# zhen6618/EPRecon

Hardware: AMD Instinct MI355X
Metric: fragments_per_sec (higher is better)
Workload: dtype f32

## Files before the change

### eprecon_amd/_lib.py

```python
import ctypes
import os

import torch

_HERE = os.path.dirname(os.path.abspath(__file__))
LIB_PATH = os.environ.get("EPRECON_LIB_PATH") or os.path.join(_HERE, "libeprecon_hip.so")

_c = ctypes
_vp, _i, _i64, _f, _sz = _c.c_void_p, _c.c_int, _c.c_int64, _c.c_float, _c.c_size_t

SIGNATURES = {
    "eprecon_abi_version": (_i, []),
    "eprecon_build_arch": (_c.c_char_p, []),
    "eprecon_back_project_workspace_bytes": (_sz, [_i64, _i, _i, _i, _i, _i, _i]),
    "eprecon_back_project_async": (_i, [_vp, _i64, _vp, _i, _f, _vp, _i, _vp, _i, _i, _i, _i, _i, _i,
                                        _vp, _vp, _vp, _vp, _vp, _vp, _vp, _vp, _sz, _vp]),
    "eprecon_back_project": (_i, [_vp, _i64, _vp, _i, _f, _vp, _i, _vp, _i, _i, _i, _i, _i, _i, _i,
                                  _vp, _vp, _vp, _vp, _vp, _vp, _vp, _vp, _vp, _sz, _vp]),
    "eprecon_profile_gather_kernel": (_c.c_char_p, []),
    "eprecon_hash_capacity": (_c.c_uint32, [_i64]),
    "eprecon_hash_table_bytes": (_sz, [_c.c_uint32]),
    "eprecon_hash_build_async": (_i, [_vp, _i64, _i, _vp, _c.c_uint32, _vp]),
    "eprecon_hash_build_dn_async": (_i, [_vp, _i64, _vp, _i, _vp, _c.c_uint32, _vp]),
    "eprecon_hash_query_async": (_i, [_vp, _c.c_uint32, _vp, _i64, _i, _vp, _vp]),
# ... 13 lines not shown
    "eprecon_transpose_map_async": (_i, [_vp, _i64, _vp, _i, _vp, _vp]),
    "eprecon_sparse_conv_async": (_i, [_vp, _i64, _i, _vp, _i, _i64, _vp, _i, _i, _vp, _vp, _i, _i, _i, _vp]),
    "eprecon_conv_bn_partial_bytes": (_sz, [_i64, _i]),
    "eprecon_sparse_conv_fused_async": (_i, [_vp, _i64, _i, _vp, _i, _i64, _vp, _i, _i, _vp, _vp, _i, _vp, _i, _i, _i,
                                             _vp, _vp]),
    "eprecon_conv_desc_async": (_i, [_vp, _vp]),
    "eprecon_exclusive_scan_async": (_i, [_vp, _i64, _vp, _vp, _vp, _vp]),
    "eprecon_conv_desc_partial_rows": (_i64, [_vp]),
    "eprecon_bn_acc_words": (_sz, [_i]),
    "eprecon_conv_desc_takes_bn_acc": (_i, [_vp]),
    "eprecon_batchnorm_acc_affine_async": (_i, [_vp, _i, _i, _i, _f, _vp, _vp, _vp]),
    "eprecon_affine_rows_acc_async": (_i, [_vp, _i64, _i, _i, _vp, _i, _i, _f, _i, _vp, _i, _vp]),
    "eprecon_affine_rows_res_async": (_i, [_vp, _i64, _i, _i, _vp, _vp, _vp, _i, _i, _vp, _i, _vp]),
    "eprecon_batchnorm_finalize_affine_async": (_i, [_vp, _i64, _i, _vp, _vp, _f, _vp, _vp, _vp]),
    "eprecon_affine_rows_async": (_i, [_vp, _i64, _i, _i, _vp, _vp, _i, _vp, _i, _vp]),
    "eprecon_pixel_map_async": (_i, [_i, _i, _i, _i, _vp, _vp]),
    "eprecon_batchnorm_apply_workspace_bytes": (_sz, [_i]),
    "eprecon_batchnorm_apply_partials_async": (_i, [_vp, _i64, _i, _i, _vp, _i64, _vp, _vp, _f, _vp, _i, _i, _vp, _i,
                                                    _vp, _vp, _vp, _sz, _vp]),
    "eprecon_batchnorm_apply_partials_res_async": (_i, [_vp, _i64, _i, _i, _vp, _i64, _vp, _vp, _f, _vp, _i, _vp, _vp, _i, _vp,
                                                        _i, _vp, _sz, _vp]),
    "eprecon_batchnorm_workspace_bytes": (_sz, [_i64, _i]),
    "eprecon_batchnorm_train_async": (_i, [_vp, _i64, _i, _i, _vp, _vp, _f, _vp, _i, _i, _vp, _i, _vp, _vp,
                                           _vp, _sz, _vp]),
    "eprecon_rowwise_layernorm_async": (_i, [_vp, _i64, _i, _i, _vp, _i, _vp, _vp, _f, _i, _i, _vp, _i, _vp]),
    "eprecon_init_select_workspace_bytes": (_sz, [_i, _i]),
    "eprecon_init_select_async": (_i, [_vp, _vp, _i64, _f, _i, _i, _i, _vp, _vp, _vp, _sz, _vp]),
    "eprecon_upsample_async": (_i, [_vp, _i, _vp, _i64, _i, _i, _vp, _vp, _vp]),
    "eprecon_aligned_coords_async": (_i, [_vp, _i64, _vp, _i, _f, _vp, _vp, _vp]),
    "eprecon_point_quantize_async": (_i, [_vp, _i64, _f, _vp, _vp, _vp]),
# ... 155 lines not shown
                ("residual", ctypes.c_void_p), ("ld_res", ctypes.c_int),
                ("out", ctypes.c_void_p), ("ld_out", ctypes.c_int),
                ("relu", ctypes.c_int), ("accumulate", ctypes.c_int),
                ("in_scale", ctypes.c_void_p), ("in_shift", ctypes.c_void_p), ("in_relu", ctypes.c_int),
                ("res_scale", ctypes.c_void_p), ("res_shift", ctypes.c_void_p), ("res_relu", ctypes.c_int),
                ("bn_partial", ctypes.c_void_p),
                ("ln", ctypes.c_int), ("ln_gamma", ctypes.c_void_p), ("ln_beta", ctypes.c_void_p),
                ("ln_eps", ctypes.c_float), ("ln_post_relu", ctypes.c_int),
                ("img_h", ctypes.c_int), ("img_w", ctypes.c_int), ("img_maps", ctypes.c_int),
                ("vox_rank", ctypes.c_void_p), ("grid_x", ctypes.c_int), ("grid_y", ctypes.c_int), ("grid_z", ctypes.c_int),
                ("packed_weight", ctypes.c_void_p), ("packed_weight16", ctypes.c_void_p),
                ("workspace", ctypes.c_void_p), ("workspace_bytes", ctypes.c_size_t),
                ("bn_acc", ctypes.c_void_p), ("bn_acc_ld", ctypes.c_int), ("bn_acc_c0", ctypes.c_int),
                ("bn_gamma", ctypes.c_void_p), ("bn_beta", ctypes.c_void_p),
                ("in_acc", ctypes.c_void_p), ("in_acc_ld", ctypes.c_int), ("in_acc_c0", ctypes.c_int),
                ("in_eps", ctypes.c_float), ("in_affine_scratch", ctypes.c_void_p)]


class GruStageDesc(ctypes.Structure):
    _fields_ = [("map", ctypes.c_void_p), ("target_map", ctypes.c_void_p),
                ("cur_coords", ctypes.c_void_p), ("cur_feat", ctypes.c_void_p), ("n_cur", ctypes.c_int64), ("ld_cur", ctypes.c_int),
                ("dim", ctypes.c_int), ("interval", ctypes.c_int), ("activity_mode", ctypes.c_int),
                ("rel", ctypes.c_int32 * 3),
                ("tsdf_gt", ctypes.c_void_p), ("occ_gt", ctypes.c_void_p),
                ("origin", ctypes.c_void_p), ("w2ac", ctypes.c_void_p),
                ("voxel_size", ctypes.c_float), ("resolution", ctypes.c_float),
                ("ch_voxel", ctypes.c_int), ("batch_index", ctypes.c_int),
                ("capacity", ctypes.c_int64),
                ("updated", ctypes.c_void_p), ("out_coords", ctypes.c_void_p), ("r_coords", ctypes.c_void_p),
                ("hx_voxel", ctypes.c_void_p), ("hx_image", ctypes.c_void_p), ("tsdf_target", ctypes.c_void_p),
                ("scaled1", ctypes.c_void_p), ("vox1", ctypes.c_void_p), ("inverse1", ctypes.c_void_p), ("uniq1", ctypes.c_void_p),
# ... 187 lines not shown
```

### eprecon_amd/csrc/conv_common.hpp

```cpp
#pragma once
#include "common.hpp"

namespace epconv {

struct ConvParams {
    const float *x;
    const int32_t *nbr;
    const float *w;
    const float *bias;
    float *out;
    int n_out, K, Cin, Cout, ld_x, ld_out;
    int64_t x_bytes;
    int relu;
    int accumulate;
    const float *res;
    int ld_res;
    float *bn_partial;
    const float *in_scale, *in_shift;
    int in_relu;
    const float *res_scale, *res_shift;
    int res_relu;
    int ln;
    const float *ln_gamma, *ln_beta;
    float ln_eps;
// ... 2 lines not shown
    int flex_partial;
    const int32_t *vox_rank;
    int gx, gy, gz;
    const float *wq;
    const float *wq16;
    int debug;
    int splitk_pipe;
    void *ws;
    size_t ws_bytes;
    long long *bn_acc;
    int bn_acc_ld, bn_acc_c0;
    const float *bn_gamma, *bn_beta;
    const long long *in_acc;
    int in_acc_ld, in_acc_c0;
    float in_eps;
};

constexpr int kBnCopies = 8, kBnWords = 7;
#ifndef EP_BN_ABL
#define EP_BN_ABL 0
#endif

__device__ __forceinline__ void bn_limbs(double x, long long &l0, long long &l1, long long &l2)
{
    const double v = x * 1099511627776.0;
    const double hi = floor(v * (1.0 / 1099511627776.0));
    l0 = (long long)(v - hi * 1099511627776.0);
    const long long h = (long long)hi;
    l1 = h & ((1ll << 40) - 1);
    l2 = h >> 40;
// ... 90 lines not shown
```

### eprecon_amd/csrc/grid_ops.hip

```cpp
#include "common.hpp"

namespace {
using namespace ep;

constexpr int kSelThreads = 1024;

__global__ __launch_bounds__(256) void init_mark_kernel(const float *logit, const int4 *coords, int n, float thr,
                                                        int batch, int D, int cell, unsigned char *marks)
{
    const int i = blockIdx.x * 256 + threadIdx.x;
    if (i >= n) return;
    const int4 c = coords[i];
    if (c.x < 0 || c.x >= batch) return;
    const float sig = 1.0f / (1.0f + expf(-logit[i]));
    if (sig > thr) {
        const int x = c.y / cell, y = c.z / cell, z = c.w / cell;
        if (x >= 0 && x < D && y >= 0 && y < D && z >= 0 && z < D) marks[(size_t)c.x * D * D * D + (x * D + y) * D + z] = 1;
    }
}

__device__ __forceinline__ uint32_t box_columns(const uint32_t *vol, int D, int x, int y, bool erode, uint32_t zmask)
{
    uint32_t r = erode ? zmask : 0u;
    for (int dx = -1; dx <= 1; ++dx)
// ... 128 lines not shown
        hipLaunchKernelGGL(upsample_coords_kernel, dim3((unsigned)ceil_div(n * 8, 256)), dim3(256), 0, st,
                           reinterpret_cast<const int4 *>(coords), (int)n, interval,
                           reinterpret_cast<int4 *>(up_coords));
        EP_LAUNCH_CHECK();
    }
    if (channels > 0) {
        if (!feat || !up_feat || ld_feat < channels) return EPRECON_ERR_ARG;
        const size_t total = (size_t)n * 8 * channels;
        hipLaunchKernelGGL(upsample_feat_kernel, dim3((unsigned)ceil_div((int64_t)total, 256)), dim3(256), 0,
                           st, feat, (int)n, channels, ld_feat, up_feat);
        EP_LAUNCH_CHECK();
    }
    return EPRECON_OK;
}

}

namespace {
__global__ __launch_bounds__(256) void upsample2x_nhwc_kernel(const float4 *in, float4 *out, int n, int h, int w,
                                                              int c4)
{
    const size_t e = (size_t)blockIdx.x * 256 + threadIdx.x;
    const size_t total = (size_t)n * 4 * h * w * c4;
    if (e >= total) return;
    const int c = (int)(e % c4);
    size_t r = e / c4;
    const int ox = (int)(r % (2 * w));
    r /= 2 * w;
    const int oy = (int)(r % (2 * h));
    const int img = (int)(r / (2 * h));
// ... 163 lines not shown
```

### eprecon_amd/csrc/sparse_conv.hip

```cpp
#include <stdio.h>
#include <stdlib.h>
#include <string.h>

#include "common.hpp"
#include "conv_common.hpp"

namespace {
using namespace ep;
using namespace epconv;

typedef float f32x16 __attribute__((ext_vector_type(16)));


template <int TN>
__device__ __forceinline__ void stage_weights(float *dst, const float *w, int row0, int row_end, int stride,
                                              int ncols, int rows, int tid)
{
    const int total = rows * TN;
    if (stride == TN && ncols >= TN && (reinterpret_cast<uintptr_t>(w) & 15) == 0) {
        const float4 *src = reinterpret_cast<const float4 *>(w + (size_t)row0 * stride);
        float4 *d4 = reinterpret_cast<float4 *>(dst);
        const int valid4 = max(0, min(rows, row_end - row0)) * (TN / 4);
#pragma unroll 4
        for (int e = tid; e < total / 4; e += 256) d4[e] = e < valid4 ? src[min(e, max(valid4 - 1, 0))] : make_float4(0.f, 0.f, 0.f, 0.f);
// ... 1967 lines not shown
        EP_LAUNCH_CHECK();
    }
    return rc;
}

int conv_dispatch_inner(ConvParams &p, int64_t n_in, hipStream_t st)
{
    {
        const int kind = conv3d_kind(p);
        if (kind != kD3None) {
            g_last_conv_kernel = kind == kD3Narrow ? "conv3d_tile_narrow_kernel" : "conv3d_tile16_kernel";
            return kind == kD3Tile16 ? launch_conv3d_16(p, st) : launch_conv3d_single_column(p, st);
        }
        if (!p.nbr && p.K != 1) return EPRECON_ERR_ARG;
    }
    const bool direct2d = p.K == 9 && direct16_ok(p);
    if (!direct2d) {
        int nt, nch;
        int64_t blocks;
        if (conv2d_tile_ok(p, &nt, &nch, &blocks)) {
            g_last_conv_kernel = "conv2d_tile_kernel";
            switch (nch) {
                case 1: return launch_conv2d_tile<1>(p, st);
                case 2: return launch_conv2d_tile<2>(p, st);
                case 3: return launch_conv2d_tile<3>(p, st);
                case 4: return launch_conv2d_tile<4>(p, st);
                default: return launch_conv2d_tile<5>(p, st);
            }
        }
    }
// ... 137 lines not shown
extern "C" size_t eprecon_conv_bn_partial_bytes(int64_t n_out, int cout)
{
    return (size_t)ep::ceil_div(n_out > 0 ? n_out : 1, (int64_t)128) * 3 * (size_t)(cout > 0 ? cout : 1) * sizeof(float);
}

static int conv_check_and_run(ConvParams &p, int64_t n_in, int64_t n_out, void *stream)
{
    if (!p.x || !p.w || !p.out || n_in < 0 || n_out < 0 || p.K <= 0 || p.K > 64 || p.Cin <= 0 || p.Cout <= 0 ||
        p.ld_x < p.Cin || p.ld_out < p.Cout || (p.res && p.ld_res < p.Cout))
        return EPRECON_ERR_ARG;
    if (!p.nbr && !p.vox_rank && p.K != 1) return EPRECON_ERR_ARG;
    if (!p.nbr && n_in != n_out) return EPRECON_ERR_ARG;
    if ((p.in_scale == nullptr) != (p.in_shift == nullptr) || (p.res_scale == nullptr) != (p.res_shift == nullptr))
        return EPRECON_ERR_ARG;
    if (p.Cout > 4096 || n_out > 0x7fffffff) return EPRECON_ERR_UNSUPPORTED;
    if (n_out == 0) return EPRECON_OK;
    p.n_out = (int)n_out;
    p.x_bytes = n_in > 0 ? ((n_in - 1) * (int64_t)p.ld_x + ((p.Cin + 3) & ~3)) * 4 : 0;
    return conv_dispatch(p, n_in, (hipStream_t)stream);
}

static void params_from_desc(ConvParams &p, const eprecon_conv_desc *d)
{
    p.x = d->x; p.nbr = d->nbr; p.w = d->weight; p.bias = d->bias; p.out = d->out;
    p.K = d->kvol; p.Cin = d->cin; p.Cout = d->cout; p.ld_x = d->ld_x; p.ld_out = d->ld_out;
    p.relu = d->relu; p.accumulate = d->accumulate;
    p.res = d->residual; p.ld_res = d->ld_res; p.bn_partial = d->bn_partial;
    p.in_scale = d->in_scale; p.in_shift = d->in_shift; p.in_relu = d->in_relu;
    p.res_scale = d->res_scale; p.res_shift = d->res_shift; p.res_relu = d->res_relu;
    p.ln = d->ln; p.ln_gamma = d->ln_gamma; p.ln_beta = d->ln_beta; p.ln_eps = d->ln_eps;
    p.ln_post_relu = d->ln_post_relu;
    p.img_h = d->img_h; p.img_w = d->img_w; p.img_maps = d->img_maps;
    p.vox_rank = d->vox_rank; p.gx = d->grid_x; p.gy = d->grid_y; p.gz = d->grid_z; p.wq = d->packed_weight;
    p.wq16 = d->packed_weight16;
    p.ws = d->workspace; p.ws_bytes = d->workspace_bytes;
    p.flex_partial = 1;
    p.bn_acc = d->bn_acc; p.bn_acc_ld = d->bn_acc_ld; p.bn_acc_c0 = d->bn_acc_c0; p.bn_gamma = d->bn_gamma; p.bn_beta = d->bn_beta;
    p.in_acc = d->in_acc; p.in_acc_ld = d->in_acc_ld; p.in_acc_c0 = d->in_acc_c0; p.in_eps = d->in_eps;
}

extern "C" int eprecon_batchnorm_acc_affine_async(const long long *acc, int acc_ld, int acc_c0, int channels, float eps,
                                                  float *scale_out, float *shift_out, void *stream);

static bool bn_acc_family(const ConvParams &p) { return conv3d_kind(p) == 0; }

extern "C" size_t eprecon_bn_acc_words(int ld)
{
    return ld > 0 ? (size_t)epconv::kBnCopies * ld * epconv::kBnWords + (size_t)(2 * ld + 1) / 2 : 0;
}

extern "C" int eprecon_conv_desc_takes_bn_acc(const eprecon_conv_desc *d)
{
    if (!d || d->n_out <= 0) return 0;
// ... 81 lines not shown
```

### eprecon_amd/csrc/sparse_conv_direct_impl.hpp

```cpp
#pragma once
#include <stdlib.h>

#include <atomic>
#include <type_traits>

#include "common.hpp"
#include "conv_common.hpp"

namespace epconv {
namespace {
using namespace ep;

constexpr int kRT = 2;

#ifndef EP_DIRECT_ABL
#define EP_DIRECT_ABL 0
#endif

__device__ __forceinline__ float relu_nc(float x)
{
    float r;
    asm("v_max_f32 %0, 0, %1" : "=v"(r) : "v"(x));
    return r;
}
// ... 66 lines not shown
            if (colok[t] && orow[r] >= 0) {
                val = acc[r >> 2][t][r & 3] + b;
                if (p.relu) val = fmaxf(val, 0.0f);
                if (p.res) {
                    float rv = p.res[(size_t)orow[r] * p.ld_res + col];
                    if (p.res_scale) {
                        rv = fmaf(rv, rs, rb);
                        if (p.res_relu) rv = fmaxf(rv, 0.0f);
                    }
                    val += rv;
                }
            }
            v[t][r] = val;
        }
    }
    if (p.ln) {
        const float inv_c = 1.0f / (float)p.Cout;
#pragma unroll
        for (int r = 0; r < NR; ++r) {
            float sum = 0.0f;
#pragma unroll
            for (int t = 0; t < CT; ++t) sum += v[t][r];
#pragma unroll
            for (int m = 8; m > 0; m >>= 1) sum += __shfl_xor(sum, m);
            const float mean = sum * inv_c;
            float sq = 0.0f;
#pragma unroll
            for (int t = 0; t < CT; ++t) {
                const float d = colok[t] ? v[t][r] - mean : 0.0f;
                v[t][r] = d;
                sq = fmaf(d, d, sq);
// ... 840 lines not shown
        if (n <= 0) n = 256;
    }
    return n;
}

static bool persist_enabled()
{
    const char *e = getenv("EPRECON_CONV_PERSIST");
    return e && e[0] == '1';
}

constexpr int kPersistMinRows = 8192;

static bool persist_ok(const ConvParams &p)
{
    if (!persist_enabled() || (p.Cin + 15) / 16 > 6) return false;
    if (p.Cout - 16 * ((p.Cout + 15) / 16 - 1) <= 8 && !tail8_enabled()) return false;
    if (p.bn_partial && !p.flex_partial) return false;
    if (persist_lds_bytes(p) > kLdsBytes) return false;
    {
        const int kch = (p.Cin + 15) / 16, ct = (p.Cout + 15) / 16;
        const bool tail = p.Cout - 16 * (ct - 1) <= 8;
        if (kch * ((tail ? ct - 1 : ct) * 1024 + (tail ? 512 : 0)) > 4864) return false;
    }
    return p.n_out >= kPersistMinRows;
}

template <int CT, int KCH, bool TAIL>
int launch_persist(const ConvParams &p, hipStream_t st)
{
    static bool attr_set = false;
// ... 119 lines not shown
```

### eprecon_amd/dense2d.py

```python
import ctypes
import os

import torch

from . import _lib
from . import sparse as SP


class PixelGrid:
    _cache = {}

    def __init__(self, maps, height, width, device):
        self.maps, self.height, self.width, self.device = maps, height, width, device
        self.n = maps * height * width
        self._nbr = {}

    @classmethod
    def get(cls, maps, height, width, device):
        key = (maps, height, width, str(device))
        g = cls._cache.get(key)
        if g is None:
            g = cls._cache[key] = cls(maps, height, width, device)
        return g

# ... 192 lines not shown
    n, c = rows.shape
    if out is None:
        out = torch.empty((n, c), dtype=torch.float32, device=rows.device)
    if act.scale is None and c <= 512:
        _lib.check(_lib.load().eprecon_affine_rows_acc_async(
            rows.data_ptr(), n, c, rows.stride(0), act.acc.block.data_ptr(), act.acc.ld, act.acc.c0, float(act.eps), int(act.relu),
            out.data_ptr(), out.stride(0), _lib.current_stream()), "eprecon_affine_rows_acc_async")
        return out
    act.affine()
    _lib.check(_lib.load().eprecon_affine_rows_async(
        rows.data_ptr(), n, c, rows.stride(0), act.scale.data_ptr(), act.shift.data_ptr(), int(act.relu),
        out.data_ptr(), out.stride(0), _lib.current_stream()), "eprecon_affine_rows_async")
    return out


def conv_bn(conv, bn, x, grid, out=None, relu=True, pre_relu=False, pre_residual=None):
    res = Act(pre_residual) if pre_residual is not None else None
    return materialize(conv_bn_act(conv, bn, Act(x), grid, relu=relu, pre_relu=pre_relu, residual=res), out=out)
```

### eprecon_amd/modules.py

```python
import math

import torch
import torch.nn as nn
import torch.nn.functional as F

from . import autograd as AG
from . import dense2d as D2
from . import sparse as SP


def recording():
    return torch.is_grad_enabled()

_SET_CACHE = []
_SET_CACHE_MAX = 8
_SET_CACHE_LOCK = __import__("threading").Lock()


def voxel_set_for(coords, stride=1):
    key = (coords.data_ptr(), coords.shape[0], coords._version, int(stride), coords.device)
    with _SET_CACHE_LOCK:
        for k, ref, vs in _SET_CACHE:
            if k == key and ref is coords:
                return vs
# ... 115 lines not shown
        self.conv6 = SubMconv3dBlock(h, h, 3, 1, 1)
        self.conv7 = SubMconv3dBlock(dim * 4, dim, 1, 1, 0)
        self.dim = dim

    def run(self, x, vset):
        d, h = self.dim, self.dim // 2
        n = x.shape[0]
        if recording():
            x1, x2 = self.conv1.run(x, vset), self.conv2.run(x, vset)
            x3 = self.conv3.run(x2, vset)
            x4 = self.conv4.run(x3, vset)
            x5 = self.conv5.run(x4, vset)
            x6 = self.conv6.run(x5, vset)
            return self.conv7.run(torch.cat([x1, x2, x3, x4, x5, x6], dim=1), vset)
        cat = torch.empty((n, 4 * d), dtype=torch.float32, device=x.device)
        self.conv1.run(x, vset, out=cat[:, 0:d])
        self.conv2.run(x, vset, out=cat[:, d:2 * d])
        self.conv3.run(cat[:, d:2 * d], vset, out=cat[:, 2 * d:2 * d + h])
        self.conv4.run(cat[:, 2 * d:2 * d + h], vset, out=cat[:, 2 * d + h:3 * d])
        self.conv5.run(cat[:, 2 * d + h:3 * d], vset, out=cat[:, 3 * d:3 * d + h])
        self.conv6.run(cat[:, 3 * d:3 * d + h], vset, out=cat[:, 3 * d + h:4 * d])
        return self.conv7.run(cat, vset)

    def forward(self, voxel_features_o, voxel_coords_bxyz, batch_size, spitial_shape):
        return self.run(voxel_features_o.contiguous(), voxel_set_for(voxel_coords_bxyz))


class SparseConv3d_Residual(nn.Module):

    def __init__(self, dim, Kernel):
        super().__init__()
        self.SConv3d = SparseSubMConv3d(dim, dim, Kernel)
        self.norm = _RowLayerNorm(dim)

    def run(self, x, vset):
        return self.SConv3d.run_ln(x, vset, self.norm, relu=True, residual=x)

    def forward(self, x, coords, spitial_shape, bs):
        return self.run(x.contiguous(), voxel_set_for(coords))

# ... 102 lines not shown

    def run_act(self, x, grid):
        d = x.rows.shape[1]
        h = d // 2
        dev = x.rows.device
        cat = torch.empty((x.rows.shape[0], 4 * d), dtype=torch.float32, device=dev)
        if D2._ARENA is not None:
            acc = D2.AccSlice.new(4 * d)
            eps = self.conv1.bn.eps
            part = lambda a, b: D2.Act(cat[:, a:b], relu=True, acc=acc.part(a, b), eps=eps)
            sl = lambda a, b: dict(out=cat[:, a:b], aff=acc.part(a, b))
        else:
            aff = torch.empty((2, 4 * d), dtype=torch.float32, device=dev)
            part = lambda a, b: D2.Act(cat[:, a:b], aff[0, a:b], aff[1, a:b], True)
            sl = lambda a, b: dict(out=cat[:, a:b], aff=(aff[0, a:b], aff[1, a:b]))
        self.conv1.run_act(x, grid, **sl(0, d))
        self.conv2.run_act(x, grid, **sl(d, 2 * d))
        self.conv3.run_act(part(d, 2 * d), grid, **sl(2 * d, 2 * d + h))
        self.conv4.run_act(part(2 * d, 2 * d + h), grid, **sl(2 * d + h, 3 * d))
        self.conv5.run_act(part(2 * d + h, 3 * d), grid, **sl(3 * d, 3 * d + h))
        self.conv6.run_act(part(3 * d, 3 * d + h), grid, **sl(3 * d + h, 4 * d))
        return self.conv7.run_act(part(0, 4 * d), grid)

    def run_rows(self, x, grid, out=None):
        return D2.materialize(self.run_act(D2.Act(x), grid), out=out)


class Fusion_Block(nn.Module):

    def __init__(self, C):
        super().__init__()
        self.conv1 = nn.Conv2d(C, C, 3, padding="same")
        self.bn1 = nn.BatchNorm2d(C)
        self.relu = nn.ReLU()
        self.conv2 = nn.Conv2d(C, C, 1, padding="same")
        self.bn2 = nn.BatchNorm2d(C)
        self.ELAN = ELAN(C)

    def forward(self, x):
        x = bn2d_train(self.bn1, self.conv1(x), relu=True)
        x = bn2d_train(self.bn2, self.conv2(x), relu=True)
        return self.ELAN(x)

    def run_rows(self, x, grid, out=None):
        a = D2.conv_bn_act(self.conv1, self.bn1, D2.Act(x), grid, relu=True)
        a = D2.conv_bn_act(self.conv2, self.bn2, a, grid, relu=True)
        return D2.materialize(self.ELAN.run_act(a, grid), out=out)


def _ln_rows(norm, y, residual=None, pre_relu=False, post_relu=False):
    if y.is_cuda and not torch.is_grad_enabled() and y.dim() == 2 and y.dtype == torch.float32 and y.is_contiguous() \
            and (residual is None or (residual.is_contiguous() and residual.dtype == torch.float32)):
        return SP.rowwise_layernorm(y, norm.weight, norm.bias, norm.eps, residual, pre_relu, post_relu, out=y)
    t = F.relu(y) if pre_relu else y
    if residual is not None:
        t = t + residual
    t = norm(t)
    return F.relu(t) if post_relu else t


_FUSED_HEADS = __import__("os").environ.get("EPRECON_FUSED_HEADS", "1") == "1"

# ... 453 lines not shown
```

### eprecon_amd/occupancy_initialization.py

```python
import os

import torch
import torch.nn as nn
import torch.nn.functional as F

from . import _lib
from . import back_project as BP
from .back_project import Back_Project, get_img_feats
from . import dense2d as D2
from . import sparse as SP
from .config import INIT_MIN_VALID
from .modules import (Conv2d_Block, Conv2d_Residual_Block, Fusion_Block, SparseSubMConv3d, Spares3dELAN,
                      TrainBatchNorm1d, _RowLayerNorm, upsample2x_bilinear)


class Occupancy_Initialization(nn.Module):
    def __init__(self, ch_initialization_all, ch_initialization_down, n_views):
        super().__init__()
        ch_all = sum(ch_initialization_all[:3])
        d = ch_initialization_down
        self.self_fusion_1x = Fusion_Block(ch_initialization_all[0])
        self.self_fusion_2x = Fusion_Block(ch_initialization_all[1])
        self.self_fusion_4x = Fusion_Block(ch_initialization_all[2])
        self.pool4x = nn.AvgPool2d(2)
# ... 47 lines not shown
        dev = rows[0].device
        grids = [D2.PixelGrid.get(v, h, w, dev) for v, c, h, w in shapes]
        g1, g2, g4 = grids
        c1, c2, c4 = (r.shape[1] for r in rows)
        cat = torch.empty((g2.n, c1 + c2 + c4), dtype=torch.float32, device=dev)
        main = torch.cuda.current_stream()
        if self._side_streams is None:
            self._side_streams = (_lib.side_stream(dev, _lib.SIDE_BRANCH_A), _lib.side_stream(dev, _lib.SIDE_BRANCH_B))
        s1, s4 = self._side_streams
        if D2.BN_ACC and self._bn_arena is None:
            self._bn_arena = D2.BnArena(dev)
        with D2.bn_pass(self._bn_arena if D2.BN_ACC else None):
            s1.wait_stream(main)
            s4.wait_stream(main)
            with torch.cuda.stream(s4):
                f4 = self.self_fusion_4x.run_rows(rows[2], g4)
                cat[:, c1 + c2:] = D2.rows_of(self.pool4x(D2.maps_of(f4, g4.maps, g4.height, g4.width)))
            with torch.cuda.stream(s1):
                f1 = self.self_fusion_1x.run_rows(rows[0], g1)
                up = upsample2x_bilinear(D2.maps_of(f1, g1.maps, g1.height, g1.width))
                cat[:, 0:c1] = D2.rows_of(up)
            self.self_fusion_2x.run_rows(rows[1], g2, out=cat[:, c1:c1 + c2])
            main.wait_stream(s1)
            main.wait_stream(s4)
            a = self.fusion_down.run_act(D2.Act(cat), g2)
            for blk in (self.post_fusion_1, self.post_fusion_2, self.post_fusion_3, self.post_fusion_4):
                a = blk.run_act(a, g2)
            return D2.maps_of(D2.materialize(a), g2.maps, g2.height, g2.width)

    def _fusion_graphed(self, views):
        key = tuple(tuple(v[0].shape) + (len(v),) for v in views) + (views[0][0].device,)
        direct = self.use_hip_conv and len(views[0]) <= 16 and all(
            m.dtype == torch.float32 and m.is_contiguous() for v in views for m in v)
        key = key + (direct,)
        entry = self._graphs.get(key)
        if entry is None:
            shapes = [(len(v),) + tuple(v[0].shape) for v in views]
# ... 89 lines not shown
```

### eprecon_amd/sparse.py

```python
import ctypes

import torch

from . import _lib


import os

def _dense3d_level():
    return int(os.environ.get("EPRECON_CONV_DENSE3D", "2"))


def _ld(t):
    assert t.dim() == 2 and t.stride(1) == 1, "row-major 2-D tensor expected"
    return t.stride(0)


class HashGrid:

    def __init__(self, n, device):
        lib = _lib.load()
        self.capacity = int(lib.eprecon_hash_capacity(int(n)))
        self.mem = torch.empty(int(lib.eprecon_hash_table_bytes(self.capacity)), dtype=torch.uint8,
                               device=device)
# ... 442 lines not shown
        out = torch.empty((n_out, cout), dtype=torch.float32, device=x.device)
    assert out.shape == (n_out, cout)
    partial = None
    if bn_partial:
        partial = torch.empty(((n_out + 127) // 128, 3, cout), dtype=torch.float32, device=x.device)
    if residual is not None:
        assert residual.shape == (n_out, cout) and residual.dtype == torch.float32
    _lib.check(lib.eprecon_sparse_conv_fused_async(
        _lib.ptr(x), x.shape[0], _ld(x), _lib.ptr(nbr), kvol, n_out, _lib.ptr(weight), cin, cout, _lib.ptr(bias),
        _lib.ptr(residual), _ld(residual) if residual is not None else 0, _lib.ptr(out), _ld(out), int(relu),
        int(accumulate), _lib.ptr(partial), _lib.current_stream()), "eprecon_sparse_conv_fused_async")
    return out, partial


def sparse_conv_ln(x, weight, nbr, bias, ln_weight, ln_bias, ln_eps, out=None, relu=False, residual=None,
                   post_relu=False):
    lib = _lib.load()
    w_owner = weight
    if weight.dim() == 2:
        weight = weight.unsqueeze(0)
    kvol, cin, cout = weight.shape
    weight = weight.contiguous()
    n_out = x.shape[0] if nbr is None else nbr.shape[1]
    assert x.shape[1] == cin and x.dtype == torch.float32 and cout <= 128
    if out is None:
        out = torch.empty((n_out, cout), dtype=torch.float32, device=x.device)
    d = _lib.ConvDesc()
    d.x, d.n_in, d.ld_x = x.data_ptr(), x.shape[0], _ld(x)
    d.kvol, d.n_out = kvol, n_out
    keep = _resolve_map(nbr, x, weight, d, ln=True, owner=w_owner)
    d.weight, d.cin, d.cout = weight.data_ptr(), cin, cout
    d.bias = None if bias is None else bias.data_ptr()
    if residual is not None:
        assert residual.shape == (n_out, cout)
        d.residual, d.ld_res = residual.data_ptr(), _ld(residual)
    d.out, d.ld_out = out.data_ptr(), _ld(out)
    d.relu = int(relu)
    d.ln = 1
    d.ln_gamma = None if ln_weight is None else ln_weight.data_ptr()
    d.ln_beta = None if ln_bias is None else ln_bias.data_ptr()
    d.ln_eps, d.ln_post_relu = float(ln_eps), int(post_relu)
    _lib.check(lib.eprecon_conv_desc_async(ctypes.byref(d), _lib.current_stream()), "eprecon_conv_desc_async")
    return out


def affine_rows(x, scale, shift, residual=None, relu=False, out=None):
    lib = _lib.load()
    n, c = x.shape
    if out is None:
        out = torch.empty((n, c), dtype=torch.float32, device=x.device)
    _lib.check(lib.eprecon_affine_rows_res_async(
        _lib.ptr(x), n, c, _ld(x), _lib.ptr(scale), _lib.ptr(shift), _lib.ptr(residual),
        _ld(residual) if residual is not None else 0, int(relu), _lib.ptr(out), _ld(out), _lib.current_stream()),
        "eprecon_affine_rows_res_async")
    return out

# ... 152 lines not shown
```

### include/eprecon_hip.h

```cpp
#ifndef EPRECON_HIP_H
#define EPRECON_HIP_H

#include <stddef.h>
#include <stdint.h>

#ifdef __cplusplus
extern "C" {
#endif

#define EPRECON_OK 0
#define EPRECON_EMPTY 1
#define EPRECON_ERR_ARG (-1)
#define EPRECON_ERR_WORKSPACE (-2)
#define EPRECON_ERR_UNSUPPORTED (-3)
#define EPRECON_ERR_HIP_BASE (-1000)

#define EPRECON_ABI_VERSION 1
int eprecon_abi_version(void);
const char *eprecon_build_arch(void);

#define EPRECON_BP_MEAN 0
#define EPRECON_BP_MEAN_DEPTH 1
#define EPRECON_BP_VARIANCE 2

// ... 85 lines not shown
    const float *bias;
    const float *residual; int ld_res;
    float *out; int ld_out;
    int relu; int accumulate;
    const float *in_scale; const float *in_shift; int in_relu;
    const float *res_scale; const float *res_shift; int res_relu;
    float *bn_partial;
    int ln; const float *ln_gamma; const float *ln_beta; float ln_eps; int ln_post_relu;
    int img_h; int img_w; int img_maps;
    const int32_t *vox_rank; int grid_x; int grid_y; int grid_z;
    const float *packed_weight;
    const float *packed_weight16;
    void *workspace; size_t workspace_bytes;
    long long *bn_acc; int bn_acc_ld; int bn_acc_c0; const float *bn_gamma; const float *bn_beta;
    const long long *in_acc; int in_acc_ld; int in_acc_c0; float in_eps; float *in_affine_scratch;
} eprecon_conv_desc;
size_t eprecon_bn_acc_words(int ld);
int eprecon_conv_desc_takes_bn_acc(const eprecon_conv_desc *desc);
int eprecon_batchnorm_acc_affine_async(const long long *acc, int acc_ld, int acc_c0, int channels, float eps, float *scale_out,
                                       float *shift_out, void *stream);
int eprecon_affine_rows_acc_async(const float *x, int64_t n, int channels, int ld_x, const long long *acc, int acc_ld, int acc_c0,
                                  float eps, int relu, float *out, int ld_out, void *stream);
int eprecon_conv_desc_async(const eprecon_conv_desc *desc, void *stream);
size_t eprecon_conv_desc_workspace_bytes(const eprecon_conv_desc *desc);
int64_t eprecon_conv_desc_partial_rows(const eprecon_conv_desc *desc);
int eprecon_batchnorm_finalize_affine_async(const float *partial, int64_t nblk, int channels, const float *gamma,
                                            const float *beta, float eps, float *scale_out, float *shift_out,
                                            void *stream);
int eprecon_affine_rows_async(const float *x, int64_t n, int channels, int ld_x, const float *scale,
                              const float *shift, int relu, float *out, int ld_out, void *stream);
// ... 279 lines not shown
    const int32_t *parent2; const int32_t *parent4;
    const void *table1; const void *table2; const void *table4;
    uint32_t capacity1; uint32_t capacity2; uint32_t capacity4;
    int32_t *offsets1; int32_t *order1; int32_t *idx4; int32_t *offsets4; int32_t *order4;
    int32_t *down12; int32_t *up21; int32_t *down24; int32_t *up42;
    int32_t *k1; int32_t *k2; int32_t *k4;
    int32_t *idx8_1; float *weight8_1; int32_t *idx8_4; float *weight8_4;
    void *workspace; size_t workspace_bytes;
} eprecon_spvcnn_geometry_desc;
size_t eprecon_spvcnn_geometry_workspace_bytes(int64_t n, int64_t n1, int64_t n4);
int eprecon_spvcnn_geometry_async(const eprecon_spvcnn_geometry_desc *desc, void *stream);

int eprecon_upsample2x_nhwc_async(const float *in, float *out, int n, int h, int w, int channels,
                                  void *stream);

size_t eprecon_sparse_conv_wgrad_workspace_bytes(int kvol, int64_t n_out, int cin, int cout);
int eprecon_sparse_conv_wgrad_async(const float *x, int ld_x, const float *dy, int ld_dy, const int32_t *nbr, int kvol,
                                    int64_t n_out, int cin, int cout, float *dweight, void *workspace,
                                    size_t workspace_bytes, void *stream);
int eprecon_invert_map_async(const int32_t *nbr, int kvol, int64_t n_out, int64_t n_in, int32_t *inv, void *stream);
int eprecon_devoxelize_backward_async(const float *dout, int ld_out, const int32_t *idx8, const float *weight8, int64_t n,
                                      int channels, int64_t n_voxels, float *dvoxel_feat, int ld_feat, void *stream);
int eprecon_devoxelize_backward_csr_async(const float *dout, int ld_out, const float *weight8, const int32_t *offsets,
                                          const int32_t *order, int64_t n_voxels, int channels, float *dvoxel_feat, int ld_feat,
                                          void *stream);
int eprecon_gather_rows_scaled_async(const float *src, int ld_src, const int32_t *idx, const float *scale, int64_t n,
                                     int channels, float *dst, int ld_dst, void *stream);
int eprecon_back_project_backward_async(const int32_t *coords_valid, int64_t n_valid, const float *origin, int batch,
                                        float voxel_size, const float *feats_nhwc, const float *krcam, int n_views,
                                        int channels, int height, int width, int mode, const float *dout, int ld_dout,
// ... 13 lines not shown
```

Before: 679.9.

## Merge sibling 1x1 ELAN convs and fuse BN-apply with resampling

The two sibling 1x1 convolutions in the sparse and 2D ELAN blocks now run as one conv with concatenated weights. In the sparse path this uses a new grouped LayerNorm mode in the direct16 kernel. A new kernel applies the pending BN affine and ReLU while doing 2x upsampling, 2x pooling or a plain copy straight into the concat buffer. This replaces separate materialize, pool/upsample and copy steps in the occupancy initialization fusion. It saves launches and memory passes, at the cost of cached merged weights and a new kernel path that disables the persistent kernel for grouped LN.

```diff
diff --git a/eprecon_amd/_lib.py b/eprecon_amd/_lib.py
--- a/eprecon_amd/_lib.py
+++ b/eprecon_amd/_lib.py
@@ -51,6 +51,7 @@
     "eprecon_affine_rows_res_async": (_i, [_vp, _i64, _i, _i, _vp, _vp, _vp, _i, _i, _vp, _i, _vp]),
     "eprecon_batchnorm_finalize_affine_async": (_i, [_vp, _i64, _i, _vp, _vp, _f, _vp, _vp, _vp]),
     "eprecon_affine_rows_async": (_i, [_vp, _i64, _i, _i, _vp, _vp, _i, _vp, _i, _vp]),
+    "eprecon_bn_resample_rows_async": (_i, [_vp, _i, _vp, _vp, _i, _i, _i, _i, _i, _i, _vp, _i, _vp]),
     "eprecon_pixel_map_async": (_i, [_i, _i, _i, _i, _vp, _vp]),
     "eprecon_batchnorm_apply_workspace_bytes": (_sz, [_i]),
     "eprecon_batchnorm_apply_partials_async": (_i, [_vp, _i64, _i, _i, _vp, _i64, _vp, _vp, _f, _vp, _i, _i, _vp, _i,
@@ -236,7 +237,7 @@
                 ("bn_acc", ctypes.c_void_p), ("bn_acc_ld", ctypes.c_int), ("bn_acc_c0", ctypes.c_int),
                 ("bn_gamma", ctypes.c_void_p), ("bn_beta", ctypes.c_void_p),
                 ("in_acc", ctypes.c_void_p), ("in_acc_ld", ctypes.c_int), ("in_acc_c0", ctypes.c_int),
-                ("in_eps", ctypes.c_float), ("in_affine_scratch", ctypes.c_void_p)]
+                ("in_eps", ctypes.c_float), ("in_affine_scratch", ctypes.c_void_p), ("ln_group", ctypes.c_int)]
 
 
 class GruStageDesc(ctypes.Structure):
diff --git a/eprecon_amd/csrc/conv_common.hpp b/eprecon_amd/csrc/conv_common.hpp
--- a/eprecon_amd/csrc/conv_common.hpp
+++ b/eprecon_amd/csrc/conv_common.hpp
@@ -40,6 +40,7 @@
     const long long *in_acc;
     int in_acc_ld, in_acc_c0;
     float in_eps;
+    int ln_group;
 };
 
 constexpr int kBnCopies = 8, kBnWords = 7;
diff --git a/eprecon_amd/csrc/grid_ops.hip b/eprecon_amd/csrc/grid_ops.hip
--- a/eprecon_amd/csrc/grid_ops.hip
+++ b/eprecon_amd/csrc/grid_ops.hip
@@ -166,6 +166,71 @@
     return EPRECON_OK;
 }
 
+}
+
+namespace {
+__device__ __forceinline__ float bn_tap(const float *x, size_t row, int ld_x, int c, float sc, float sh, int relu)
+{
+    float v = fmaf(x[row * ld_x + c], sc, sh);
+    if (relu) v = fmaxf(v, 0.0f);
+    return v;
+}
+
+__global__ __launch_bounds__(256) void bn_resample_rows_kernel(const float *x, int ld_x, const float *scale, const float *shift,
+                                                               int relu, int mode, int maps, int h, int w, int c, float *out,
+                                                               int ld_out)
+{
+    const int oh = mode == 1 ? 2 * h : (mode == 2 ? h / 2 : h), ow = mode == 1 ? 2 * w : (mode == 2 ? w / 2 : w);
+    const size_t e = (size_t)blockIdx.x * 256 + threadIdx.x;
+    const size_t total = (size_t)maps * oh * ow * c;
+    if (e >= total) return;
+    const int ch = (int)(e % c);
+    size_t r = e / c;
+    const int ox = (int)(r % ow);
+    r /= ow;
+    const int oy = (int)(r % oh);
+    const size_t img = r / oh;
+    const size_t base = img * h * w;
+    const float sc = scale ? scale[ch] : 1.0f, sh = scale ? shift[ch] : 0.0f;
+    float o;
+    if (mode == 1) {
+        const float sx = fmaxf(((float)ox + 0.5f) * 0.5f - 0.5f, 0.0f);
+        const float sy = fmaxf(((float)oy + 0.5f) * 0.5f - 0.5f, 0.0f);
+        const int x0 = (int)sx, y0 = (int)sy;
+        const int x1 = min(x0 + 1, w - 1), y1 = min(y0 + 1, h - 1);
+        const float lx = sx - (float)x0, ly = sy - (float)y0;
+        const float a = bn_tap(x, base + (size_t)y0 * w + x0, ld_x, ch, sc, sh, relu);
+        const float b = bn_tap(x, base + (size_t)y0 * w + x1, ld_x, ch, sc, sh, relu);
+        const float d = bn_tap(x, base + (size_t)y1 * w + x0, ld_x, ch, sc, sh, relu);
+        const float f = bn_tap(x, base + (size_t)y1 * w + x1, ld_x, ch, sc, sh, relu);
+        const float w00 = (1.0f - ly) * (1.0f - lx), w01 = (1.0f - ly) * lx, w10 = ly * (1.0f - lx), w11 = ly * lx;
+        o = w00 * a + w01 * b + w10 * d + w11 * f;
+    } else if (mode == 2) {
+        float sum = 0.0f;
+        for (int dy = 0; dy < 2; ++dy)
+            for (int dx = 0; dx < 2; ++dx)
+                sum += bn_tap(x, base + (size_t)(2 * oy + dy) * w + (2 * ox + dx), ld_x, ch, sc, sh, relu);
+        o = sum / 4.0f;
+    } else {
+        o = bn_tap(x, base + (size_t)oy * w + ox, ld_x, ch, sc, sh, relu);
+    }
+    out[((img * oh + oy) * ow + ox) * (size_t)ld_out + ch] = o;
+}
+}
+
+extern "C" int eprecon_bn_resample_rows_async(const float *x, int ld_x, const float *scale, const float *shift, int relu, int mode,
+                                              int maps, int h, int w, int channels, float *out, int ld_out, void *stream)
+{
+    if (!x || !out || (scale == nullptr) != (shift == nullptr) || mode < 0 || mode > 2 || maps <= 0 || h <= 0 || w <= 0 ||
+        channels <= 0 || ld_x < channels || ld_out < channels || (mode == 2 && (h % 2 || w % 2)))
+        return EPRECON_ERR_ARG;
+    const int64_t opix = mode == 1 ? (int64_t)4 * h * w : (mode == 2 ? (int64_t)(h / 2) * (w / 2) : (int64_t)h * w);
+    const int64_t total = (int64_t)maps * opix * channels;
+    if (total > 0x7fffffffll * 256) return EPRECON_ERR_UNSUPPORTED;
+    hipLaunchKernelGGL(bn_resample_rows_kernel, dim3((unsigned)ceil_div(total, (int64_t)256)), dim3(256), 0, (hipStream_t)stream, x,
+                       ld_x, scale, shift, relu, mode, maps, h, w, channels, out, ld_out);
+    EP_LAUNCH_CHECK();
+    return EPRECON_OK;
 }
 
 namespace {
diff --git a/eprecon_amd/csrc/sparse_conv.hip b/eprecon_amd/csrc/sparse_conv.hip
--- a/eprecon_amd/csrc/sparse_conv.hip
+++ b/eprecon_amd/csrc/sparse_conv.hip
@@ -2005,6 +2005,10 @@
         }
         if (!p.nbr && p.K != 1) return EPRECON_ERR_ARG;
     }
+    if (p.ln_group) {
+        g_last_conv_kernel = "spconv_direct16_kernel";
+        return launch_direct16(p, st);
+    }
     const bool direct2d = p.K == 9 && direct16_ok(p);
     if (!direct2d) {
         int nt, nch;
@@ -2172,9 +2176,11 @@
     if ((p.in_scale == nullptr) != (p.in_shift == nullptr) || (p.res_scale == nullptr) != (p.res_shift == nullptr))
         return EPRECON_ERR_ARG;
     if (p.Cout > 4096 || n_out > 0x7fffffff) return EPRECON_ERR_UNSUPPORTED;
+    if (p.ln_group && (p.ln_group < 0 || p.ln_group % 16 || p.Cout % p.ln_group || !p.ln)) return EPRECON_ERR_ARG;
     if (n_out == 0) return EPRECON_OK;
     p.n_out = (int)n_out;
     p.x_bytes = n_in > 0 ? ((n_in - 1) * (int64_t)p.ld_x + ((p.Cin + 3) & ~3)) * 4 : 0;
+    if (p.ln_group && (p.K != 1 || p.nbr || !direct16_ok(p))) return EPRECON_ERR_UNSUPPORTED;
     return conv_dispatch(p, n_in, (hipStream_t)stream);
 }
 
@@ -2195,6 +2201,7 @@
     p.flex_partial = 1;
     p.bn_acc = d->bn_acc; p.bn_acc_ld = d->bn_acc_ld; p.bn_acc_c0 = d->bn_acc_c0; p.bn_gamma = d->bn_gamma; p.bn_beta = d->bn_beta;
     p.in_acc = d->in_acc; p.in_acc_ld = d->in_acc_ld; p.in_acc_c0 = d->in_acc_c0; p.in_eps = d->in_eps;
+    p.ln_group = d->ln_group == d->cout ? 0 : d->ln_group;
 }
 
 extern "C" int eprecon_batchnorm_acc_affine_async(const long long *acc, int acc_ld, int acc_c0, int channels, float eps,
diff --git a/eprecon_amd/csrc/sparse_conv_direct_impl.hpp b/eprecon_amd/csrc/sparse_conv_direct_impl.hpp
--- a/eprecon_amd/csrc/sparse_conv_direct_impl.hpp
+++ b/eprecon_amd/csrc/sparse_conv_direct_impl.hpp
@@ -104,7 +104,43 @@
             v[t][r] = val;
         }
     }
-    if (p.ln) {
+    if (!PERWAVE && p.ln && p.ln_group) {
+        const int gt = p.ln_group >> 4;
+        const float inv_g = 1.0f / (float)p.ln_group;
+#pragma unroll
+        for (int r = 0; r < NR; ++r) {
+            float s[CT], mean[CT], sq[CT];
+#pragma unroll
+            for (int t = 0; t < CT; ++t) {
+                s[t] = 0.0f;
+#pragma unroll
+                for (int t2 = 0; t2 < CT; ++t2)
+                    if (t2 / gt == t / gt) s[t] += v[t2][r];
+#pragma unroll
+                for (int m = 8; m > 0; m >>= 1) s[t] += __shfl_xor(s[t], m);
+                mean[t] = s[t] * inv_g;
+            }
+#pragma unroll
+            for (int t = 0; t < CT; ++t) v[t][r] = colok[t] ? v[t][r] - mean[t] : 0.0f;
+#pragma unroll
+            for (int t = 0; t < CT; ++t) {
+                sq[t] = 0.0f;
+#pragma unroll
+                for (int t2 = 0; t2 < CT; ++t2)
+                    if (t2 / gt == t / gt) sq[t] = fmaf(v[t2][r], v[t2][r], sq[t]);
+#pragma unroll
+                for (int m = 8; m > 0; m >>= 1) sq[t] += __shfl_xor(sq[t], m);
+            }
+#pragma unroll
+            for (int t = 0; t < CT; ++t) {
+                const int col = 16 * t + l16;
+                const float inv = 1.0f / sqrtf(sq[t] * inv_g + p.ln_eps);
+                float y = fmaf(v[t][r] * inv, (p.ln_gamma && colok[t]) ? p.ln_gamma[col] : 1.0f, (p.ln_beta && colok[t]) ? p.ln_beta[col] : 0.0f);
+                if (p.ln_post_relu) y = fmaxf(y, 0.0f);
+                v[t][r] = y;
+            }
+        }
+    } else if (p.ln) {
         const float inv_c = 1.0f / (float)p.Cout;
 #pragma unroll
         for (int r = 0; r < NR; ++r) {
@@ -975,7 +1011,7 @@
 
 static bool persist_ok(const ConvParams &p)
 {
-    if (!persist_enabled() || (p.Cin + 15) / 16 > 6) return false;
+    if (!persist_enabled() || (p.Cin + 15) / 16 > 6 || p.ln_group) return false;
     if (p.Cout - 16 * ((p.Cout + 15) / 16 - 1) <= 8 && !tail8_enabled()) return false;
     if (p.bn_partial && !p.flex_partial) return false;
     if (persist_lds_bytes(p) > kLdsBytes) return false;
diff --git a/eprecon_amd/dense2d.py b/eprecon_amd/dense2d.py
--- a/eprecon_amd/dense2d.py
+++ b/eprecon_amd/dense2d.py
@@ -230,6 +230,22 @@
     return out
 
 
+RESAMPLE_NONE, RESAMPLE_UP2, RESAMPLE_POOL2 = 0, 1, 2
+
+
+def resample_into(act, grid, mode, out):
+    rows = act.rows
+    n, c = rows.shape
+    assert n == grid.n and rows.stride(1) == 1 and out.stride(1) == 1 and out.shape[1] == c
+    f = {RESAMPLE_NONE: 1, RESAMPLE_UP2: 4, RESAMPLE_POOL2: 0.25}[mode]
+    assert out.shape[0] == int(n * f)
+    scale, shift = act.affine() if (act.scale is not None or act.acc is not None) else (None, None)
+    _lib.check(_lib.load().eprecon_bn_resample_rows_async(
+        rows.data_ptr(), rows.stride(0), _dptr(scale), _dptr(shift), int(act.relu), mode, grid.maps, grid.height, grid.width, c,
+        out.data_ptr(), out.stride(0), _lib.current_stream()), "eprecon_bn_resample_rows_async")
+    return out
+
+
 def conv_bn(conv, bn, x, grid, out=None, relu=True, pre_relu=False, pre_residual=None):
     res = Act(pre_residual) if pre_residual is not None else None
     return materialize(conv_bn_act(conv, bn, Act(x), grid, relu=relu, pre_relu=pre_relu, residual=res), out=out)
diff --git a/eprecon_amd/modules.py b/eprecon_amd/modules.py
--- a/eprecon_amd/modules.py
+++ b/eprecon_amd/modules.py
@@ -1,4 +1,5 @@
 import math
+import os
 
 import torch
 import torch.nn as nn
@@ -153,8 +154,12 @@
             x6 = self.conv6.run(x5, vset)
             return self.conv7.run(torch.cat([x1, x2, x3, x4, x5, x6], dim=1), vset)
         cat = torch.empty((n, 4 * d), dtype=torch.float32, device=x.device)
-        self.conv1.run(x, vset, out=cat[:, 0:d])
-        self.conv2.run(x, vset, out=cat[:, d:2 * d])
+        if 2 * d <= SP.DIRECT_MAX_COUT and n >= SP.K1_DIRECT_MIN_ROWS and x.is_cuda and os.environ.get("EPRECON_CONV_DIRECT") != "0":
+            w, b, g, be = self._siblings()
+            SP.sparse_conv_ln(x, w, None, b, g, be, self.conv1.ln.eps, out=cat[:, 0:2 * d], post_relu=True, ln_group=d)
+        else:
+            self.conv1.run(x, vset, out=cat[:, 0:d])
+            self.conv2.run(x, vset, out=cat[:, d:2 * d])
         self.conv3.run(cat[:, d:2 * d], vset, out=cat[:, 2 * d:2 * d + h])
         self.conv4.run(cat[:, 2 * d:2 * d + h], vset, out=cat[:, 2 * d + h:3 * d])
         self.conv5.run(cat[:, 2 * d + h:3 * d], vset, out=cat[:, 3 * d:3 * d + h])
@@ -163,6 +168,19 @@
 
     def forward(self, voxel_features_o, voxel_coords_bxyz, batch_size, spitial_shape):
         return self.run(voxel_features_o.contiguous(), voxel_set_for(voxel_coords_bxyz))
+
+    def _siblings(self):
+        a, b = self.conv1, self.conv2
+        assert a.ln.eps == b.ln.eps
+        params = (a.conv.weight, b.conv.weight, a.conv.bias, b.conv.bias, a.ln.weight, b.ln.weight, a.ln.bias, b.ln.bias)
+        tag = tuple((t._version, t.data_ptr()) for t in params)
+        hit = getattr(self, "_eprecon_merged", None)
+        if hit is None or hit[0] != tag:
+            with torch.no_grad():
+                hit = (tag, (torch.cat([a.conv.weight, b.conv.weight], dim=2).contiguous(), torch.cat([a.conv.bias, b.conv.bias]),
+                             torch.cat([a.ln.weight, b.ln.weight]), torch.cat([a.ln.bias, b.ln.bias])))
+            self._eprecon_merged = hit
+        return hit[1]
 
 
 class SparseConv3d_Residual(nn.Module):
@@ -295,13 +313,31 @@
             aff = torch.empty((2, 4 * d), dtype=torch.float32, device=dev)
             part = lambda a, b: D2.Act(cat[:, a:b], aff[0, a:b], aff[1, a:b], True)
             sl = lambda a, b: dict(out=cat[:, a:b], aff=(aff[0, a:b], aff[1, a:b]))
-        self.conv1.run_act(x, grid, **sl(0, d))
-        self.conv2.run_act(x, grid, **sl(d, 2 * d))
+        if 2 * d <= SP.DIRECT_MAX_COUT and x.rows.shape[0] >= D2.K1_DIRECT_2D_MIN_ROWS:
+            w, bias, gamma, beta = self._siblings()
+            D2.conv_bn_launch(w, bias, gamma, beta, self.conv1.bn.eps, 1, x, grid, relu=True, **sl(0, 2 * d))
+        else:
+            self.conv1.run_act(x, grid, **sl(0, d))
+            self.conv2.run_act(x, grid, **sl(d, 2 * d))
         self.conv3.run_act(part(d, 2 * d), grid, **sl(2 * d, 2 * d + h))
         self.conv4.run_act(part(2 * d, 2 * d + h), grid, **sl(2 * d + h, 3 * d))
         self.conv5.run_act(part(2 * d + h, 3 * d), grid, **sl(3 * d, 3 * d + h))
         self.conv6.run_act(part(3 * d, 3 * d + h), grid, **sl(3 * d + h, 4 * d))
         return self.conv7.run_act(part(0, 4 * d), grid)
+
+    def _siblings(self):
+        a, b = self.conv1, self.conv2
+        assert a.bn.eps == b.bn.eps
+        params = (a.conv.weight, b.conv.weight, a.conv.bias, b.conv.bias, a.bn.weight, b.bn.weight, a.bn.bias, b.bn.bias)
+        tag = tuple((t._version, t.data_ptr()) for t in params)
+        hit = getattr(self, "_eprecon_merged", None)
+        if hit is None or hit[0] != tag:
+            with torch.no_grad():
+                hit = (tag, (torch.cat([D2.packed_weight(a.conv), D2.packed_weight(b.conv)], dim=2).contiguous(),
+                             torch.cat([a.conv.bias, b.conv.bias]), torch.cat([a.bn.weight, b.bn.weight]),
+                             torch.cat([a.bn.bias, b.bn.bias])))
+            self._eprecon_merged = hit
+        return hit[1]
 
     def run_rows(self, x, grid, out=None):
         return D2.materialize(self.run_act(D2.Act(x), grid), out=out)
@@ -323,10 +359,13 @@
         x = bn2d_train(self.bn2, self.conv2(x), relu=True)
         return self.ELAN(x)
 
-    def run_rows(self, x, grid, out=None):
+    def run_act(self, x, grid):
         a = D2.conv_bn_act(self.conv1, self.bn1, D2.Act(x), grid, relu=True)
         a = D2.conv_bn_act(self.conv2, self.bn2, a, grid, relu=True)
-        return D2.materialize(self.ELAN.run_act(a, grid), out=out)
+        return self.ELAN.run_act(a, grid)
+
+    def run_rows(self, x, grid, out=None):
+        return D2.materialize(self.run_act(x, grid), out=out)
 
 
 def _ln_rows(norm, y, residual=None, pre_relu=False, post_relu=False):
diff --git a/eprecon_amd/occupancy_initialization.py b/eprecon_amd/occupancy_initialization.py
--- a/eprecon_amd/occupancy_initialization.py
+++ b/eprecon_amd/occupancy_initialization.py
@@ -85,13 +85,10 @@
             s1.wait_stream(main)
             s4.wait_stream(main)
             with torch.cuda.stream(s4):
-                f4 = self.self_fusion_4x.run_rows(rows[2], g4)
-                cat[:, c1 + c2:] = D2.rows_of(self.pool4x(D2.maps_of(f4, g4.maps, g4.height, g4.width)))
+                D2.resample_into(self.self_fusion_4x.run_act(rows[2], g4), g4, D2.RESAMPLE_POOL2, cat[:, c1 + c2:])
             with torch.cuda.stream(s1):
-                f1 = self.self_fusion_1x.run_rows(rows[0], g1)
-                up = upsample2x_bilinear(D2.maps_of(f1, g1.maps, g1.height, g1.width))
-                cat[:, 0:c1] = D2.rows_of(up)
-            self.self_fusion_2x.run_rows(rows[1], g2, out=cat[:, c1:c1 + c2])
+                D2.resample_into(self.self_fusion_1x.run_act(rows[0], g1), g1, D2.RESAMPLE_UP2, cat[:, 0:c1])
+            D2.resample_into(self.self_fusion_2x.run_act(rows[1], g2), g2, D2.RESAMPLE_NONE, cat[:, c1:c1 + c2])
             main.wait_stream(s1)
             main.wait_stream(s4)
             a = self.fusion_down.run_act(D2.Act(cat), g2)
diff --git a/eprecon_amd/sparse.py b/eprecon_amd/sparse.py
--- a/eprecon_amd/sparse.py
+++ b/eprecon_amd/sparse.py
@@ -480,7 +480,7 @@
 
 
 def sparse_conv_ln(x, weight, nbr, bias, ln_weight, ln_bias, ln_eps, out=None, relu=False, residual=None,
-                   post_relu=False):
+                   post_relu=False, ln_group=0):
     lib = _lib.load()
     w_owner = weight
     if weight.dim() == 2:
@@ -506,6 +506,7 @@
     d.ln_gamma = None if ln_weight is None else ln_weight.data_ptr()
     d.ln_beta = None if ln_bias is None else ln_bias.data_ptr()
     d.ln_eps, d.ln_post_relu = float(ln_eps), int(post_relu)
+    d.ln_group = int(ln_group)
     _lib.check(lib.eprecon_conv_desc_async(ctypes.byref(d), _lib.current_stream()), "eprecon_conv_desc_async")
     return out
 
diff --git a/include/eprecon_hip.h b/include/eprecon_hip.h
--- a/include/eprecon_hip.h
+++ b/include/eprecon_hip.h
@@ -123,6 +123,7 @@
     void *workspace; size_t workspace_bytes;
     long long *bn_acc; int bn_acc_ld; int bn_acc_c0; const float *bn_gamma; const float *bn_beta;
     const long long *in_acc; int in_acc_ld; int in_acc_c0; float in_eps; float *in_affine_scratch;
+    int ln_group;
 } eprecon_conv_desc;
 size_t eprecon_bn_acc_words(int ld);
 int eprecon_conv_desc_takes_bn_acc(const eprecon_conv_desc *desc);
@@ -432,6 +433,9 @@
 int eprecon_upsample2x_nhwc_async(const float *in, float *out, int n, int h, int w, int channels,
                                   void *stream);
 
+int eprecon_bn_resample_rows_async(const float *x, int ld_x, const float *scale, const float *shift, int relu, int mode,
+                                   int maps, int h, int w, int channels, float *out, int ld_out, void *stream);
+
 size_t eprecon_sparse_conv_wgrad_workspace_bytes(int kvol, int64_t n_out, int cin, int cout);
 int eprecon_sparse_conv_wgrad_async(const float *x, int ld_x, const float *dy, int ld_dy, const int32_t *nbr, int kvol,
                                     int64_t n_out, int cin, int cout, float *dweight, void *workspace,
```

Result: no change. 686.6, median of 6 (+1.0%).
